# Basant1861/MPC-MMD

Hardware: AMD Instinct MI355X
Metric: MPC optimizer steps/s (batch=1024,H=30,obs_samp=500) @1/2/4/8 GPU; % HBM roofline (higher is better)
Workload: dtype f32; 1 GPU; static obs, mmd_opt, batch=1024 rollouts, H=30, num_obs=10, obs_samples=484 (n=22, M=n^2); cost=mmd_opt, global_batch=1024, num_batch=1024, num_prime=30, num_obs=10, num_reduced=22, noise=gaussian, parallelism=config-sharded x1

## Files before the change

### mpc-mmd_amd/csrc/betacem_common.hpp

```cpp
#pragma once
#include <type_traits>

#include "block.hpp"
#include "kernels.hpp"

namespace mpcmmd {

namespace {

#ifdef MPCMMD_OPAQUE_TIDX
DEVI unsigned tidx() {
  unsigned t = threadIdx.x;
  asm volatile("" : "+v"(t));
  return t;
}
#else
DEVI unsigned tidx() { return threadIdx.x; }
#endif

constexpr int kF = 22;
constexpr int kNew = kBetaSamples - kBetaElite;
constexpr int kThreads = 512;
constexpr double kSqrt20 = 4.47213595499957927704;
constexpr double kRidge = 0.05;
constexpr double kInvRidge = 20.0;

HDI int first_sample(int tb) { return tb > 0 ? kBetaElite : 0; }

#define kconst __attribute__((address_space(4)))
typedef float f2 __attribute__((ext_vector_type(2)));

typedef double d4 __attribute__((ext_vector_type(4)));
DEVI d4 mfma64(double a, double b, d4 c) { return __builtin_amdgcn_mfma_f64_16x16x4f64(a, b, c, 0, 0, 0); }

constexpr int kXcds = 8;
constexpr int kCUs = 256;
constexpr int kKerWaves = 16;
constexpr int kDirWaves = 4;
constexpr int kLptBins = 128;
constexpr double kSeriesAMax = 1.0;
constexpr float kNegLog2e = -1.44269504088896340736f;
constexpr size_t kLdsBudget = 160 * 1024 - 1024;

template <int V = 1, class F>
void with_dist_blocks(int M, F&& f) {
  if constexpr (V == 16) {
    f(std::integral_constant<int, 16>{});
  } else {
    if ((dist_stride(M) >> 8) == V) f(std::integral_constant<int, V>{});
    else with_dist_blocks<V + 1>(M, f);
  }
}

struct LdsTake {
  size_t o = 0;
  HDI size_t operator()(size_t bytes) {
    const size_t at = o;
    o = (o + bytes + 15) & ~size_t(15);
    return at;
  }
};

struct KerLds {
  size_t sel, csg, csd, tri, urank, urow, misc, scratch, total;
};
HDI KerLds ker_lds(int M, int n, size_t scratch) {
  KerLds L{};
  LdsTake take;
  L.sel = take(size_t(kBetaSamples) * n * 2);
  L.csg = take(size_t(kBetaSamples) * 4);
  L.csd = take(size_t(kBetaSamples) * 8);
  L.tri = take(size_t(n) * (n - 1));
  L.urank = take(size_t(M) * 2);
  L.urow = take(size_t(M) * 2);
  L.misc = take(32 * 4);
  L.scratch = take(scratch);
  L.total = take.o;
  return L;
}
HDI size_t ker_sample_bytes(int n) { return size_t(kKerWaves) * n * kFeatStride * 4; }
HDI size_t ker_tab_bytes(int U) { return ((size_t(U) * (U - 1) / 2 * 4 + 15) & ~size_t(15)) + size_t(U) * kFeatStride * 4; }
constexpr size_t kKerTabBytes = 55 * 1024;
constexpr size_t kKerRecBytes = 64 * 1024;
HDI size_t ker_scratch(int M, int n, int tb) {
  size_t sc = ker_sample_bytes(n);
  size_t rec = size_t(M) * kMomStride * 4;
  if (rec > kKerRecBytes) rec = kKerRecBytes;
  if (rec > sc) sc = rec;
  if (tb > 0 && kKerTabBytes > sc) sc = kKerTabBytes;
  return sc;
}

struct DirLds {
  size_t sel, csg, pairs, ulist, ustart, order, bins, misc, scratch, total;
};
HDI DirLds dir_lds(int M, int n) {
  DirLds L{};
  LdsTake take;
  L.sel = take(size_t(kBetaSamples) * n * 2);
  L.csg = take(size_t(kBetaSamples) * 4);
  L.pairs = take(size_t(kBetaSamples) * n * 2);
  L.ulist = take(size_t(M) * 2);
  L.ustart = take(size_t(M + 1) * 2);
  L.order = take(size_t(M) * 2);
  L.bins = take(kLptBins * 4);
  L.misc = take(32 * 4);
  L.scratch = take(size_t(M) * 10);
  L.total = take.o;
  return L;
}

struct EliteLds {
  size_t Gb, misc, carry, ublk, total;
};
constexpr int kUPitch = 12;
HDI EliteLds elite_lds(int M1, int waves = kThreads / 64) {
  EliteLds L{};
  const int nblk = (M1 + 15) / 16;
  L.Gb = 0;
  L.misc = (size_t(nblk) * 66 * 8 + 15) & ~size_t(15);
  L.carry = L.misc + 1024;
  L.ublk = (L.carry + size_t(kBetaElite) * (2 * kMaxReduced + 2) * 4 + 15) & ~size_t(15);
  L.total = L.ublk + size_t(waves) * 16 * kUPitch * 8;
  return L;
}

HDI size_t gen_lds_bytes(int M) { return size_t(pos_pad(M)) * (2 * kGenRow + 1) * 8 + 16 * 8; }
HDI size_t tblk_lds_bytes(int M) { return size_t(pos_pad(M) >> 4) * 4 * 64 * 8; }

}

}
```

### mpc-mmd_amd/csrc/betacem_elite.hpp

```cpp
#pragma once
#include "betacem_common.hpp"

namespace mpcmmd {

namespace {

HDI int sym11(int a, int c) { return a * 11 - a * (a - 1) / 2 + (c - a); }
HDI int sym11i(int a, int c) { return a <= c ? sym11(a, c) : sym11(c, a); }

DEVI void belite_body(const Params& p, int tb, int b, char* smem) {
  const int M = p.M, M1 = M + 1, n = p.n, tid = tidx();
  const EliteLds C = elite_lds(M1, blockDim.x >> 6);
  double* Gb = reinterpret_cast<double*>(smem + C.Gb);
  int* elite = reinterpret_cast<int*>(smem + C.misc);
  int* info = elite + 16;
  float* cst = reinterpret_cast<float*>(info + 16);
  float* sig_new = cst + kBetaSamples;
  uint32_t* ckey = reinterpret_cast<uint32_t*>(sig_new + 12);
  const float* costs = p.bcost + size_t(b) * kBetaSamples;
  if (tid < kBetaSamples) {
    const float c = costs[tid];
    cst[tid] = c;
    ckey[tid] = sort_key(c);
  }
  if (tid == 0) {
    info[0] = -1;
    info[1] = 0;
  }
  __syncthreads();
  if (tid < kBetaSamples) {
    const uint32_t ks = ckey[tid];
    const uint4* k4 = reinterpret_cast<const uint4*>(ckey);
    int r = 0;
#pragma unroll
    for (int k = 0; k < kBetaSamples / 4; ++k) {
      const uint4 v = k4[k];
      r += int(v.x < ks || (v.x == ks && 4 * k < tid)) + int(v.y < ks || (v.y == ks && 4 * k + 1 < tid)) +
           int(v.z < ks || (v.z == ks && 4 * k + 2 < tid)) + int(v.w < ks || (v.w == ks && 4 * k + 3 < tid));
    }
    if (r < kBetaElite) elite[r] = tid;
    if (cst[tid] != cst[tid]) {
      atomicOr(&info[1], 1);
      atomicMin(reinterpret_cast<unsigned*>(&info[0]), unsigned(tid));
    }
  }
  __syncthreads();
  const int imin = info[1] ? info[0] : elite[0];
  if (tid == 0) {
    p.res_beta[size_t(b) * kBetaIters + tb] = info[1] ? __int_as_float(0x7fc00000) : cst[elite[0]];
    double es = 0.0;
    for (int q = 0; q < kBetaElite; ++q) es += double(cst[elite[q]]);
    p.btrace[size_t(b) * kBetaIters + tb] = float(es);
  }
  if (tb < kBetaIters - 1) {
    int* csel = reinterpret_cast<int*>(smem + C.carry);
    float* ctop = reinterpret_cast<float*>(csel + kBetaElite * n);
    float* csig = ctop + kBetaElite * n;
    float* ccost = csig + kBetaElite;
    const size_t rb = size_t(b) * kBetaSamples;
    for (int i = tid; i < kBetaElite * n; i += blockDim.x) {
      const int q = i / n, k = i - q * n;
      const size_t src = (rb + elite[q]) * n + k;
      csel[i] = p.bsel[src];
      ctop[i] = p.btop[src];
    }
    if (tid < kBetaElite) {
      csig[tid] = p.bsig[rb + elite[tid]];
      ccost[tid] = cst[elite[tid]];
    }
    __syncthreads();
    for (int i = tid; i < kBetaElite * n; i += blockDim.x) {
      p.bsel[rb * n + i] = csel[i];
      p.btop[rb * n + i] = ctop[i];
    }
    if (tid < kBetaElite) {
      p.bsig[rb + tid] = csig[tid];
      p.bcost[rb + tid] = ccost[tid];
    }
  }
  const float* Eold = p.belite + (size_t(tb & 1) * p.Bt + b) * kBetaElite * M1;
  float* Enew = p.belite + (size_t((tb + 1) & 1) * p.Bt + b) * kBetaElite * M1;
  const int ys = ygen_stride(M);
  const float* Y = p.ygen + size_t(b) * kBzCols * ys;
  const double rs10 = 1.0 / sqrt(10.0);
  double* gen = p.gen + size_t(b) * pos_pad(M) * kGenStride;
  const int nblk = (M1 + 15) / 16;
  const int span = ((nblk * 16 + 63) / 64) * 64;
  for (int j = tid; j < span; j += blockDim.x) {
    const bool valid = j < M1;
    double u[kBetaElite], mean;
    {
      float v[kBetaElite];
      double s = 0.0;
      const int jc = min(j, M);
#pragma unroll
      for (int q = 0; q < kBetaElite; ++q) {
        const int e = elite[q];
        const float* src = tb == 0 ? p.beta_z0 + size_t(e) * M1
                                   : (e < kBetaElite ? Eold + size_t(e) * M1 : Y + size_t(e - kBetaElite) * ys);
        v[q] = src[jc];
      }
#pragma unroll
      for (int q = 0; q < kBetaElite; ++q) {
        float x = v[q];
        if (tb == 0) {
          x = float(kSqrt20 * double(x));
          if (j == M) x = fmaxf(x, 0.01f);
        }
        x = valid ? x : 0.0f;
        if (valid) {
          Enew[size_t(q) * M1 + j] = x;
          if (j == M) sig_new[q] = x;
        }
        v[q] = x;
        s = s + double(x);
      }
      const double m = s / double(kBetaElite);
#pragma unroll
      for (int q = 0; q < kBetaElite; ++q) u[q] = valid ? (double(v[q]) - m) * rs10 : 0.0;
      mean = valid ? double(float(m)) : 0.0;
    }
    double* ub = reinterpret_cast<double*>(smem + C.ublk) + (tid >> 6) * 16 * kUPitch;
    const int lane = tid & 63, r = lane & 15, h = lane >> 4;
#pragma unroll
    for (int k = 0; k < 4; ++k) {
      const int blk = (j >> 6) * 4 + k;
      if ((lane >> 4) == k) {
#pragma unroll
        for (int q = 0; q < kBetaElite; ++q) ub[(lane & 15) * kUPitch + q] = u[q];
        ub[(lane & 15) * kUPitch + kGenMean] = mean;
      }
      wave_sync();
      d4 G = d4{0.0, 0.0, 0.0, 0.0};
#pragma unroll
      for (int st = 0; st < 4; ++st) {
        const double x = r < 11 ? ub[(4 * st + h) * kUPitch + r] : 0.0;
        G = mfma64(x, x, G);
      }
#pragma unroll
      for (int i = 0; i < 3; ++i) {
        const int e = lane + 64 * i, row = e / kGenRow, q = e - row * kGenRow;
        const int pos = blk * 16 + row;
        if (pos < M1) gen[gen_uplane(pos_pad(M)) + size_t(pos) * kGenRow + q] = ub[row * kUPitch + q];
      }
      wave_sync();
#pragma unroll
      for (int i = 0; i < 4; ++i) {
        const int a = h + 4 * i;
        if (blk < nblk && a <= r && r < 11) Gb[blk * 66 + sym11(a, r)] = G[i];
      }
    }
  }
  __syncthreads();
  if (tid < 66) {
    int a = 0, c = tid;
    while (c >= 11 - a) {
      c -= 11 - a;
      ++a;
    }
    c += a;
    double acc = a == c ? 1.0 : 0.0;
    double* ph = p.phib + size_t(b) * nblk * 66;
#pragma unroll 8
    for (int blk = 0; blk < nblk; ++blk) {
      const double g = Gb[blk * 66 + tid];
      ph[blk * 66 + tid] = acc;
      acc = fma(g, kInvRidge, acc);
    }
  }
  if (tb == kBetaIters - 1) {
    const int* bsel = p.bsel + (size_t(b) * kBetaSamples + imin) * n;
    for (int i = tid; i < n; i += blockDim.x) {
      p.bestsel[size_t(b) * n + i] = bsel[i];
      p.beta[size_t(b) * n + i] = p.btop[(size_t(b) * kBetaSamples + imin) * n + i];
    }
    if (tid == 0) {
      p.bimin[b] = imin;
      if (imin < kBetaElite) p.sigma[b] = sig_new[imin];
    }
  }
}

DEVI double rcp_nr(double d) {
  double y = __builtin_amdgcn_rcp(d);
  y = fma(y, fma(-d, y, 1.0), y);
  return fma(y, fma(-d, y, 1.0), y);
}
DEVI double rsq_nr(double d) {
  double y = __builtin_amdgcn_rsq(d);
#pragma unroll
  for (int it = 0; it < 2; ++it) {
    const double e = fma(-(d * y), y, 1.0);
    y = fma(0.5 * y, e, y);
  }
  return y;
}

DEVI void bgen_wave(const Params& p, int b, int blk, double* xl) {
  const int M = p.M, M1 = M + 1, nblk = (M1 + 15) / 16, Pp = pos_pad(M);
  const int lane = tidx() & 63, r = lane & 15, h = lane >> 4;
  double* gen = p.gen + size_t(b) * Pp * kGenStride;
  double* gm = p.genm + size_t(b) * Pp;
  const int j0 = blk * 16;
  d4 A;
  double U[3];
  const double* Gb = p.phib + (size_t(b) * nblk + blk) * 66;
#pragma unroll
  for (int i = 0; i < 4; ++i) {
    const int a = h + 4 * i;
    A[i] = a < 11 && r < 11 ? Gb[sym11i(min(a, 10), min(r, 10))] : 0.0;
  }
#pragma unroll
  for (int s = 0; s < 3; ++s) {
    const int f = 4 * s + h;
    U[s] = f < 11 && j0 + r < M1 ? gen[gen_uplane(Pp) + size_t(j0 + r) * kGenRow + f] : 0.0;
  }
#pragma unroll
  for (int k = 0; k < 11; ++k) {
    if (r == k) {
#pragma unroll
      for (int i = 0; i < 4; ++i) xl[h + 4 * i] = A[i];
    }
    wave_sync();
    const double d = xl[k], cr = xl[r];
    double ci[4];
#pragma unroll
    for (int i = 0; i < 4; ++i) ci[i] = xl[h + 4 * i];
    wave_sync();
    const double id = rcp_nr(d);
#pragma unroll
    for (int i = 0; i < 4; ++i) {
      const int a = h + 4 * i;
      A[i] = a == k ? (r == k ? -id : cr * id) : (r == k ? ci[i] * id : A[i] - (ci[i] * cr) * id);
    }
  }
  const d4 zero = d4{0.0, 0.0, 0.0, 0.0};
#pragma unroll
  for (int i = 0; i < 4; ++i) A[i] = -A[i];
  d4 V = zero, G = zero;
#pragma unroll
  for (int s = 0; s < 3; ++s) V = mfma64(A[s], U[s], V);
#pragma unroll
  for (int s = 0; s < 3; ++s) G = mfma64(U[s], V[s], G);
#pragma unroll
  for (int i = 0; i < 4; ++i)
    if (h + 4 * i == r) G[i] = G[i] + kRidge;
#pragma unroll
  for (int k = 0; k < 16; ++k) {
    if (r == k) {
#pragma unroll
      for (int i = 0; i < 4; ++i) {
        xl[h + 4 * i] = G[i];
        xl[16 + h + 4 * i] = V[i];
      }
    }
    wave_sync();
    const double d = xl[k], gr = xl[r];
    double gi[4], vi[4];
#pragma unroll
    for (int i = 0; i < 4; ++i) {
      gi[i] = xl[h + 4 * i];
      vi[i] = xl[16 + h + 4 * i];
    }
    wave_sync();
    const double rl = rsq_nr(d);
    const double lr = r > k ? gr * rl : 0.0;
    double wk[4];
#pragma unroll
    for (int i = 0; i < 4; ++i) {
      const double li = h + 4 * i > k ? gi[i] * rl : 0.0;
      wk[i] = vi[i] * rl;
      G[i] = G[i] - li * lr;
      V[i] = V[i] - wk[i] * lr;
    }
    const int j = j0 + k;
    if (r == k && j < M1) {
      double* g = gen + size_t(j) * kGenRow + kGenW;
#pragma unroll
      for (int i = 0; i < 3; ++i) g[h + 4 * i] = h + 4 * i < 11 ? wk[i] : 0.0;
      if (h == 0) gm[j] = d * rl;
    }
  }
}

DEVI void bsigma_body(const Params& p, int tb, int b, double* red) {
  const int M = p.M, tid = tidx();
  const int imin = p.bimin[b];
  const double* gen = p.gen + size_t(b) * pos_pad(M) * kGenStride;
  {
    const float* z = p.beta_z + size_t(tb) * pos_pad(M) * kBzCols;
    const int si = imin - kBetaElite;
    double part[11];
#pragma unroll
    for (int a = 0; a < 11; ++a) part[a] = 0.0;
    for (int j = tid; j < M && tid < kThreads; j += kThreads) {
      const double zj = double(z[bz_index(j, si)]);
#pragma unroll
      for (int a = 0; a < 11; ++a) part[a] += gen[size_t(j) * kGenRow + kGenW + a] * zj;
    }
#pragma unroll
    for (int a = 0; a < 11; ++a) {
      part[a] = wave_total(part[a]);
    }
    __syncthreads();
    if ((tid & 63) == 0 && tid < kThreads)
#pragma unroll
      for (int a = 0; a < 11; ++a) red[(tid >> 6) * 11 + a] = part[a];
    __syncthreads();
    if (tid == 0) {
      const double* g = gen + size_t(M) * kGenRow;
      const double* gu = g + gen_uplane(pos_pad(M));
      double d = 0.0;
      for (int a = 0; a < 11; ++a) {
        double sa = 0.0;
        for (int w2 = 0; w2 < kThreads / 64; ++w2) sa += red[w2 * 11 + a];
        d += gu[a] * sa;
      }
      const double zM = z[bz_index(M, si)];
      const float yM = float((gu[kGenMean] + p.genm[size_t(b) * pos_pad(M) + M] * zM) + d);
      p.sigma[b] = fmaxf(yM, 0.01f);
    }
  }
}

}

}
```

### mpc-mmd_amd/csrc/betacem_sample.hpp

```cpp
#pragma once
#include "betacem_common.hpp"

namespace mpcmmd {

namespace {

constexpr int kSampleTiles = kBzCols / 16;
static_assert(kBzCols >= kNew, "sample tiles");
constexpr int kChunkWavesMax = 12;
HDI int sample_chunk(int nblk) {
  int cl = nblk <= 8 ? 4 : 8;
  while ((nblk + cl - 1) / cl > kChunkWavesMax) cl <<= 1;
  return cl;
}
template <int TPW>
constexpr int sample_waves() {
  static_assert(kSampleTiles % TPW == 0, "tiles per wave");
  return kSampleTiles / TPW;
}

template <int TPW>
struct SampleBlock {
  double wA[4];
  double wX[3];
  double uX[3];
  double L;
  float z[TPW][4];
};

template <int TPW>
DEVI void load_block(SampleBlock<TPW>& q, const double* G, const double* GU, const double* gm, const float* z, int p0,
                     int s0, int r, int h) {
#pragma unroll
  for (int k = 0; k < 4; ++k) q.wA[k] = G[size_t(p0 + 4 * k + h) * kGenRow + kGenW + r];
  const double* g = G + size_t(p0 + r) * kGenRow;
  const double* gu = GU + size_t(p0 + r) * kGenRow;
#pragma unroll
  for (int i = 0; i < 3; ++i) {
    q.wX[i] = g[kGenW + 4 * i + h];
    q.uX[i] = gu[4 * i + h];
  }
  q.L = gm[p0 + r];
  static_assert(TPW == 1 || TPW == kSampleTiles, "tile pairing of the normals' layout");
  if constexpr (TPW == 1) {
#pragma unroll
    for (int k = 0; k < 4; ++k) q.z[0][k] = z[bz_index(p0 + 4 * k + h, s0 + r)];
  } else {
    const float4* zb = reinterpret_cast<const float4*>(z + size_t(p0 >> 4) * (16 * kBzCols)) + r + 16 * h;
#pragma unroll
    for (int c = 0; c < 6; ++c) {
      const float4 f = zb[64 * c];
      const float fv[4] = {f.x, f.y, f.z, f.w};
#pragma unroll
      for (int w = 0; w < 4; ++w) {
        const int idx = 4 * c + w, k = idx / 6, t = idx % 6;
        q.z[t][k] = fv[w];
      }
    }
  }
}

struct SampleRsrc {
  __amdgpu_buffer_rsrc_t gen, genm, z;
  int vA, vX, vL, vZ;
  int uplane;
};
DEVI SampleRsrc sample_rsrc(const double* G, const double* gm, const float* z, int Pp, int r, int h) {
  SampleRsrc s;
  s.gen = __builtin_amdgcn_make_buffer_rsrc(const_cast<double*>(G), short(0), Pp * kGenStride * 8, 0x00020000);
  s.genm = __builtin_amdgcn_make_buffer_rsrc(const_cast<double*>(gm), short(0), Pp * 8, 0x00020000);
  s.z = __builtin_amdgcn_make_buffer_rsrc(const_cast<float*>(z), short(0), Pp * kBzCols * 4, 0x00020000);
  s.vA = (h * kGenRow + kGenW + r) * 8;
  s.vX = (r * kGenRow + h) * 8;
  s.vL = r * 8;
  s.vZ = (r + 16 * h) * 16;
  s.uplane = Pp * kGenRow * 8;
  return s;
}
DEVI double buf_ld_d(__amdgpu_buffer_rsrc_t rs, int voff, int soff) {
  return __builtin_bit_cast(double, __builtin_amdgcn_raw_buffer_load_b64(rs, voff, soff, 0));
}
DEVI void load_block_buf(SampleBlock<kSampleTiles>& q, const SampleRsrc& s, int p0) {
  const int sg = p0 * kGenRow * 8;
#pragma unroll
  for (int k = 0; k < 4; ++k) q.wA[k] = buf_ld_d(s.gen, s.vA + k * 4 * kGenRow * 8, sg);
#pragma unroll
  for (int i = 0; i < 3; ++i) {
    q.wX[i] = buf_ld_d(s.gen, s.vX + 32 * i, sg);
    q.uX[i] = buf_ld_d(s.gen, s.vX + 32 * i, sg + s.uplane);
  }
  q.L = buf_ld_d(s.genm, s.vL, p0 * 8);
  const int szz = (p0 >> 4) * (16 * kBzCols * 4);
#pragma unroll
  for (int c = 0; c < 6; ++c) {
    typedef float v4f __attribute__((ext_vector_type(4)));
    const v4f f = __builtin_bit_cast(v4f, __builtin_amdgcn_raw_buffer_load_b128(s.z, s.vZ + 1024 * (c % 3), szz + 3072 * (c / 3), 0));
#pragma unroll
    for (int w = 0; w < 4; ++w) {
      const int idx = 4 * c + w, k = idx / 6, t = idx % 6;
      q.z[t][k] = f[w];
    }
  }
}

template <int TPW>
DEVI void block_mfma(const SampleBlock<TPW>& cur, d4* S, const d4* Sp, d4* Y, int r, int h) {
  double zd[TPW][4];
#pragma unroll
  for (int t = 0; t < TPW; ++t)
#pragma unroll
    for (int k = 0; k < 4; ++k) zd[t][k] = double(cur.z[t][k]);
  d4 X = d4{0.0, 0.0, 0.0, 0.0};
#pragma unroll
  for (int i = 0; i < 3; ++i) X = mfma64(cur.wX[i], cur.uX[i], X);
  const d4 zero = d4{0.0, 0.0, 0.0, 0.0};
  double St[TPW][3];
#pragma unroll
  for (int t = 0; t < TPW; ++t)
#pragma unroll
    for (int k = 0; k < 3; ++k) St[t][k] = Sp[t][k] + S[t][k];
#pragma unroll
  for (int k = 0; k < 3; ++k)
#pragma unroll
    for (int t = 0; t < TPW; ++t) Y[t] = mfma64(St[t][k], cur.uX[k], k == 0 ? zero : Y[t]);
#pragma unroll
  for (int k = 0; k < 4; ++k)
#pragma unroll
    for (int t = 0; t < TPW; ++t) S[t] = mfma64(cur.wA[k], zd[t][k], S[t]);
  double T[4];
#pragma unroll
  for (int i = 0; i < 4; ++i) {
    const int k = h + 4 * i;
    T[i] = k < r ? X[i] : (k == r ? cur.L : 0.0);
  }
#pragma unroll
  for (int k = 0; k < 4; ++k)
#pragma unroll
    for (int t = 0; t < TPW; ++t) Y[t] = mfma64(zd[t][k], T[k], Y[t]);
}

HDI_CONST int tile_sample(int TPW, int s0, int t, int rho) { return TPW == 1 ? s0 + rho : 32 * (t >> 1) + 2 * rho + (t & 1); }
template <int TPW>
DEVI void block_store(const d4* Yv, float* plane, int p0, int M, int ys, int s0, int r, int h) {
  if (p0 > M) return;
#pragma unroll
  for (int t = 0; t < TPW; ++t)
#pragma unroll
    for (int i = 0; i < 4; ++i) {
      const int s = tile_sample(TPW, s0, t, h + 4 * i);
      const float v = float(Yv[t][i]);
      if (s < kNew) plane[size_t(s) * ys + p0 + r] = p0 + r == M ? fmaxf(v, 0.01f) : v;
    }
}

DEVI __amdgpu_buffer_rsrc_t ygen_rsrc(float* plane, int ys) {
  return __builtin_amdgcn_make_buffer_rsrc(plane, short(0), kBzCols * ys * 4, 0x00020000);
}
constexpr int kDropOffset = 0x7FFFFF00;
static_assert(kNew == 89, "tile 4 / 5 register 3 validity below");
DEVI void block_store_rows(const d4* Yv, __amdgpu_buffer_rsrc_t yr, int p0, int ys, int vl, int v43) {
#pragma unroll
  for (int t = 0; t < kSampleTiles; ++t)
#pragma unroll
    for (int i = 0; i < 4; ++i) {
      if (t == 5 && i == 3) continue;
      const int soff = ((32 * (t >> 1) + (t & 1) + 8 * i) * ys + p0) * 4;
      __builtin_amdgcn_raw_buffer_store_b32(__float_as_uint(float(Yv[t][i])), yr, t == 4 && i == 3 ? v43 : vl, soff, 0);
    }
}

DEVI void fold_chunk(d4& Sp, d4& S) {
#pragma unroll
  for (int k = 0; k < 3; ++k) Sp[k] = Sp[k] + S[k];
  S = d4{0.0, 0.0, 0.0, 0.0};
}

constexpr int kZAhead = 4;

DEVI void bsample_tblocks(const Params& p, const double* lg, double* Tl, int w, int W) {
  const int M = p.M, Pp = pos_pad(M), nblk = Pp >> 4;
  const int lane = tidx() & 63, r = lane & 15, h = lane >> 4;
  for (int blk = w; blk < nblk; blk += W) {
    const int p0 = blk * 16;
    const double* g = lg + size_t(p0 + r) * kGenRow;
    const double* gu = lg + gen_uplane(Pp) + size_t(p0 + r) * kGenRow;
    double wX[3], uX[3];
#pragma unroll
    for (int i = 0; i < 3; ++i) {
      wX[i] = g[kGenW + 4 * i + h];
      uX[i] = gu[4 * i + h];
    }
    const double L = lg[2 * gen_uplane(Pp) + p0 + r];
    d4 X = d4{0.0, 0.0, 0.0, 0.0};
#pragma unroll
    for (int i = 0; i < 3; ++i) X = mfma64(wX[i], uX[i], X);
#pragma unroll
    for (int i = 0; i < 4; ++i) {
      const int k = h + 4 * i;
      Tl[(size_t(blk) * 4 + i) * 64 + lane] = k < r ? X[i] : (k == r ? L : 0.0);
    }
  }
}

DEVI void bsample_unit_lds(const Params& p, int tb, int b, int tile, int chunk, const double* lg, const double* Tl) {
  const int M = p.M, Pp = pos_pad(M), nblk = Pp >> 4, cl = sample_chunk(nblk);
  const int c0 = chunk * cl, c1 = min(nblk, c0 + cl);
  const int lane = tidx() & 63, r = lane & 15, h = lane >> 4, s0 = tile * 16;
  const double* LW = lg;
  const double* LU = lg + gen_uplane(Pp);
  const float* z = p.beta_z + size_t(tb - 1) * Pp * kBzCols;
  const int ys = ygen_stride(M);
  float* plane = p.ygen + size_t(b) * kBzCols * ys;
  d4 S = d4{0.0, 0.0, 0.0, 0.0}, Sp = d4{0.0, 0.0, 0.0, 0.0};
  Sp[2] = h == 3 ? 1.0 : 0.0;
  auto zload = [&](float (&zz)[4], int c) {
#pragma unroll
    for (int k = 0; k < 4; ++k) zz[k] = z[bz_index(c * 16 + 4 * k + h, s0 + r)];
  };
  float zr[kZAhead][4];
#pragma unroll
  for (int u = 0; u < kZAhead; ++u) zload(zr[u], min(u, c1 - 1));
  const d4 zero = d4{0.0, 0.0, 0.0, 0.0};
  for (int c = 0; c < c1; c += kZAhead) {
#pragma unroll
    for (int u = 0; u < kZAhead; ++u) {
      const int cb = c + u;
      if (cb < c1) {
        const int p0 = cb * 16;
        double zd[4], wA[4];
#pragma unroll
        for (int k = 0; k < 4; ++k) {
          zd[k] = double(zr[u][k]);
          wA[k] = LW[size_t(p0 + 4 * k + h) * kGenRow + kGenW + r];
        }
        zload(zr[u], min(cb + kZAhead, c1 - 1));
        if (cb >= c0) {
          double uX[3], T[4];
#pragma unroll
          for (int i = 0; i < 3; ++i) uX[i] = LU[size_t(p0 + r) * kGenRow + 4 * i + h];
#pragma unroll
          for (int i = 0; i < 4; ++i) T[i] = Tl[(size_t(cb) * 4 + i) * 64 + lane];
          double St[3];
#pragma unroll
          for (int k = 0; k < 3; ++k) St[k] = Sp[k] + S[k];
          d4 Y = zero;
#pragma unroll
          for (int k = 0; k < 3; ++k) Y = mfma64(St[k], uX[k], k == 0 ? zero : Y);
#pragma unroll
          for (int k = 0; k < 4; ++k) S = mfma64(wA[k], zd[k], S);
#pragma unroll
          for (int k = 0; k < 4; ++k) Y = mfma64(zd[k], T[k], Y);
          block_store<1>(&Y, plane, p0, M, ys, s0, r, h);
        } else {
#pragma unroll
          for (int k = 0; k < 4; ++k) S = mfma64(wA[k], zd[k], S);
        }
        if ((cb + 1) % cl == 0) fold_chunk(Sp, S);
      }
    }
  }
}

}

}
```

### mpc-mmd_amd/csrc/k_bcem_small.hip

```cpp
#define MPCMMD_OPAQUE_TIDX 1
#include "betacem_elite.hpp"
#include "betacem_kernel.hpp"
#include "betacem_qp.hpp"
#include "betacem_sample.hpp"
#include "betacem_select.hpp"

namespace mpcmmd {

namespace {

constexpr int kSmallWaves = kKerWaves, kSmallThreads = 64 * kSmallWaves;
constexpr int kSmallSelR = 1, kSmallSelG = 32;
constexpr size_t kSmallCandBytes = size_t(64 * kSmallSelR + 8) * 8;
constexpr size_t kSmallSelBytes = kSmallCandBytes + 64 * 4 + 128 * 4;
HDI size_t small_lds(int M, int n) {
  size_t b = kSmallWaves * kSmallSelBytes + size_t(kNew) * ygen_stride(M) * 4;
  const size_t k = ker_lds(M, n, ker_scratch(M, n, 1)).total;
  const size_t d = dir_lds(M, n).total, e = elite_lds(M + 1, kSmallWaves).total;
  const size_t q = (size_t(kBetaSamples) * tri_stride(n) + kQpZeros) * 4;
  const size_t gl = ((gen_lds_bytes(M) + 15) & ~size_t(15)) + tblk_lds_bytes(M);
  b = b > q ? b : q;
  b = b > gl ? b : gl;
  b = b > k ? b : k;
  b = b > d ? b : d;
  b = b > e ? b : e;
  return b;
}

HDI size_t small_persist_off(int M, int n) { return (small_lds(M, n) + 15) & ~size_t(15); }
HDI size_t small_persist_bytes(int M) { return size_t(M) * (kMomStride + kFeatStride) * 4; }

#define SMALL_STAMP(p, slot)                                                             \
  do {                                                                                   \
    if (tidx() == 0 && (p).dbgw)                                                    \
      (p).dbgw[size_t(32768 + blockIdx.x) * 8 + (slot)] = __builtin_amdgcn_s_memrealtime(); \
  } while (0)

template <int NQ, int NP>
__global__ __launch_bounds__(kSmallThreads) void k_bcem_small(Params p0, int persist) {
  extern __shared__ __attribute__((aligned(16))) char smem[];
  const int cand = blockIdx.x;
  const int tid = tidx();
  const int w = __builtin_amdgcn_readfirstlane(tid >> 6);
  const float4* mom_l = nullptr;
  const float4* feat_l = nullptr;
  if (persist) {
    const int M = p0.M, b = p0.b0 + cand;
    float4* pm = reinterpret_cast<float4*>(smem + small_persist_off(M, p0.n));
    float4* pf = pm + M * (kMomStride / 4);
    const float4* gm = reinterpret_cast<const float4*>(p0.bmom + size_t(b) * M * kMomStride);
    const float4* gf = reinterpret_cast<const float4*>(p0.featr + size_t(b) * M * kFeatStride);
    for (int i = tid; i < M * (kMomStride / 4); i += kSmallThreads) pm[i] = gm[i];
    for (int i = tid; i < M * (kFeatStride / 4); i += kSmallThreads) pf[i] = gf[i];
    mom_l = pm;
    feat_l = pf;
    __syncthreads();
  }
  for (int tb = 0; tb < kBetaIters; ++tb) {
    typedef const Params __attribute__((address_space(4)))* KParams;
    KParams pk = (KParams)__builtin_amdgcn_kernarg_segment_ptr();
    asm volatile("" : "+s"(pk));
    const Params& p = *(const Params*)pk;
    const int b = p.b0 + cand, M = p.M, n = p.n;
    const int ntri = tri_stride(n);
    if (tb > 0) {
      if (tb == 5) SMALL_STAMP(p, 0);
      {
        const int Pp = pos_pad(M);
        const double2* gsrc = reinterpret_cast<const double2*>(p.gen + size_t(b) * Pp * kGenStride);
        const double2* msrc = reinterpret_cast<const double2*>(p.genm + size_t(b) * Pp);
        double2* dst = reinterpret_cast<double2*>(smem);
        const int ng = Pp * kGenRow, nm = Pp >> 1;
        for (int i = tid; i < ng + nm; i += kSmallThreads) dst[i] = i < ng ? gsrc[i] : msrc[i - ng];
        if (tid < 8) dst[ng + nm + tid] = double2{0.0, 0.0};
      }
      __syncthreads();
      {
        const double* lg = reinterpret_cast<const double*>(smem);
        double* Tl = reinterpret_cast<double*>(smem + ((gen_lds_bytes(M) + 15) & ~size_t(15)));
        bsample_tblocks(p, lg, Tl, w, kSmallWaves);
        __syncthreads();
        const int nblk = pos_pad(M) >> 4, units = kSampleTiles * ((nblk + sample_chunk(nblk) - 1) / sample_chunk(nblk));
        for (int u = w; u < units; u += kSmallWaves) bsample_unit_lds(p, tb, b, u % kSampleTiles, u / kSampleTiles, lg, Tl);
      }
      __syncthreads();
      if (tb == 5) SMALL_STAMP(p, 1);
      const int ys = ygen_stride(M);
      const float* Yl = reinterpret_cast<const float*>(smem + kSmallWaves * kSmallSelBytes);
      {
        const float4* src = reinterpret_cast<const float4*>(p.ygen + size_t(b) * kBzCols * ys);
        float4* dst = reinterpret_cast<float4*>(smem + kSmallWaves * kSmallSelBytes);
        for (int i = tid; i < kNew * (ys >> 2); i += kSmallThreads) dst[i] = src[i];
      }
      __syncthreads();
      char* sw = smem + size_t(w) * kSmallSelBytes;
      unsigned long long* cand_l = reinterpret_cast<unsigned long long*>(sw);
      uint32_t* lm = reinterpret_cast<uint32_t*>(sw + kSmallCandBytes);
      int* scr = reinterpret_cast<int*>(sw + kSmallCandBytes + 64 * 4);
      {
        int32_t* sel = p.bsel + size_t(b) * kBetaSamples * n;
        float* sig = p.bsig + size_t(b) * kBetaSamples;
        auto row = [&](int s) {
          const float* r = Yl + size_t(s - kBetaElite) * ys;
          return [=](int j) { return r[j]; };
        };
        const int s_lo = first_sample(tb), lane = tid & 63;
        if (s_lo + w < kBetaSamples) {
          select_walk<NQ, kSmallSelR, kSmallSelG>(row, [&](int s) { return sel + s * n; }, s_lo + w, kBetaSamples,
                                                  kSmallWaves, M, n, cand_l, lm, scr);
          for (int s2 = s_lo + w + lane * kSmallWaves; lane < 16 && s2 < kBetaSamples; s2 += 16 * kSmallWaves)
            sig[s2] = row(s2)(M);
        }
      }
    } else {
      for (int e = tid; e < kBetaSamples * n; e += kSmallThreads) p.bsel[size_t(b) * kBetaSamples * n + e] = p.sel0[e];
      for (int e = tid; e < kBetaSamples; e += kSmallThreads) p.bsig[size_t(b) * kBetaSamples + e] = p.sig0[e];
    }
    __syncthreads();
    if (tb == 5) SMALL_STAMP(p, 2);
    bkernel_body<false, true>(p, tb, cand, 0, 1, int(ker_scratch(M, n, tb)), smem, mom_l, feat_l);
    __syncthreads();
    if (tb == 5) SMALL_STAMP(p, 3);
    if (tb > 0) {
      const int total = bdirect_total(p, b, 1);
      if (total > 0) {
        bdirect_body<1, kSmallWaves>(p, tb, 1, 1, cand, 0, total, smem);
        __syncthreads();
      }
    }
    if (tb == 5) SMALL_STAMP(p, 4);
    {
      const int s_lo = first_sample(tb), per = kBetaSamples - s_lo;
      const float4* src = reinterpret_cast<const float4*>(p.bkred + (size_t(b) * kBetaSamples + s_lo) * ntri);
      float4* kl4 = reinterpret_cast<float4*>(smem);
      for (int i = tid; i < per * (ntri >> 2); i += kSmallThreads) kl4[i] = src[i];
      if (tid < kQpZeros) reinterpret_cast<float*>(smem)[per * ntri + tid] = 0.0f;
      __syncthreads();
      static_assert(kSmallThreads / 4 >= kBetaSamples, "one quad per QP");
      const int g = tid >> 2;
      const bool ok = g < per;
      const int gc = ok ? g : 0;
      bqp_solve<NP>(p, b, s_lo + gc, ok, reinterpret_cast<const float*>(smem) + size_t(gc) * ntri,
                    reinterpret_cast<const float*>(smem) + size_t(per) * ntri);
    }
    __syncthreads();
    if (tb == 5) SMALL_STAMP(p, 5);
    belite_body(p, tb, b, smem);
    __syncthreads();
    if (tb == 5) SMALL_STAMP(p, 6);
    {
      const int nblk = (M + 1 + 15) / 16;
      double* xl = reinterpret_cast<double*>(smem) + 32 * w;
      for (int blk = w; blk < nblk; blk += kSmallWaves) bgen_wave(p, b, blk, xl);
    }
    __syncthreads();
    if (tb == 5) SMALL_STAMP(p, 7);
    if (tb == kBetaIters - 1 && p.bimin[b] >= kBetaElite) {
      bsigma_body(p, tb, b, reinterpret_cast<double*>(smem));
      __syncthreads();
    }
  }
}

}

bool bcem_small_ok(const Params& p) {
  return p.gen_wave && p.M <= 256 && p.nb <= 512 && small_lds(p.M, p.n) <= kLdsBudget;
}

void launch_bcem_small(const Params& p, hipStream_t s) {
  const int n = p.n, M = p.M;
  const dim3 grid(p.nb), block(kSmallThreads);
  const size_t lp = small_persist_off(M, n) + small_persist_bytes(M);
  const int persist = lp <= kLdsBudget;
  const size_t lds = persist ? lp : small_lds(M, n);
  if (M <= 64)
    hipLaunchKernelGGL((k_bcem_small<1, 8>), grid, block, lds, s, p, persist);
  else if (M <= 128)
    hipLaunchKernelGGL((k_bcem_small<2, 12>), grid, block, lds, s, p, persist);
  else
    hipLaunchKernelGGL((k_bcem_small<4, 16>), grid, block, lds, s, p, persist);
}

}
```

### mpc-mmd_amd/csrc/k_belite.hip

```cpp
#include "betacem_elite.hpp"

namespace mpcmmd {

namespace {

__global__ __launch_bounds__(kThreads) void k_belite(Params p, int tb) {
  extern __shared__ __attribute__((aligned(16))) char smem[];
  belite_body(p, tb, p.b0 + blockIdx.x, smem);
}

DEVI void bgen_quad(const Params& p, int b, int blk, bool live) {
  const int M = p.M, M1 = M + 1, nblk = (M1 + 15) / 16;
  const int q = tidx() & 3;
  double* gen = p.gen + size_t(b) * pos_pad(M) * kGenStride;
  const double* Gb = p.phib + (size_t(b) * nblk + blk) * 66;
  double A[3][11];
#pragma unroll
  for (int i = 0; i < 3; ++i) {
    const int a = q + 4 * i;
#pragma unroll
    for (int c = 0; c < 11; ++c) A[i][c] = a < 11 ? Gb[sym11i(a, c)] : 0.0;
  }
#pragma unroll
  for (int k = 0; k < 11; ++k) {
    const int ik = k >> 2, ok = k & 3;
    const double ip = 1.0 / quad_bcast(A[ik][k], ok);
    double f[3];
#pragma unroll
    for (int i = 0; i < 3; ++i) f[i] = A[i][k];
#pragma unroll
    for (int c = 0; c < 11; ++c) {
      const double rc = c == k ? ip : quad_bcast(A[ik][c], ok) * ip;
#pragma unroll
      for (int i = 0; i < 3; ++i) {
        const bool pivot_row = q + 4 * i == k;
        A[i][c] = pivot_row ? rc : (c == k ? -f[i] * ip : fma(-f[i], rc, A[i][c]));
      }
    }
  }
  const int j0 = blk * 16, j1 = min(M1, j0 + 16);
  double un[11];
  double uon[3];
  const double* ub = gen + gen_uplane(pos_pad(M));
#pragma unroll
  for (int c = 0; c < 11; ++c) un[c] = ub[size_t(j0) * kGenRow + c];
#pragma unroll
  for (int i = 0; i < 3; ++i) uon[i] = ub[size_t(j0) * kGenRow + q + 4 * i];
  for (int j = j0; j < j1; ++j) {
    double u[11], uo[3];
#pragma unroll
    for (int c = 0; c < 11; ++c) u[c] = un[c];
#pragma unroll
    for (int i = 0; i < 3; ++i) uo[i] = uon[i];
    const int jn = min(j + 1, j1 - 1);
#pragma unroll
    for (int c = 0; c < 11; ++c) un[c] = ub[size_t(jn) * kGenRow + c];
#pragma unroll
    for (int i = 0; i < 3; ++i) uon[i] = ub[size_t(jn) * kGenRow + q + 4 * i];
    double v[3], part = 0.0;
#pragma unroll
    for (int i = 0; i < 3; ++i) {
      double s = 0.0;
#pragma unroll
      for (int c = 0; c < 11; ++c) s = fma(A[i][c], u[c], s);
      v[i] = s;
      const int a = q + 4 * i;
      part = fma(i < 2 || a < 11 ? uo[i] : 0.0, s, part);
    }
    const double uv = quad_sum(part);
    const double ljj = sqrt(kRidge + uv);
    const double rl = 1.0 / ljj;
    double w[3];
#pragma unroll
    for (int i = 0; i < 3; ++i) w[i] = v[i] * rl;
    double* g = gen + size_t(j) * kGenRow;
    if (live) {
#pragma unroll
      for (int i = 0; i < 3; ++i) g[kGenW + q + 4 * i] = q + 4 * i < 11 ? w[i] : 0.0;
      if (q == 0) p.genm[size_t(b) * pos_pad(M) + j] = ljj;
    }
#pragma unroll
    for (int c = 0; c < 11; ++c) {
      const double wc = quad_bcast(w[c >> 2], c & 3);
#pragma unroll
      for (int i = 0; i < 3; ++i) A[i][c] = fma(-w[i], wc, A[i][c]);
    }
  }
}

__global__ __launch_bounds__(256) __attribute__((amdgpu_waves_per_eu(2))) void k_bgen(Params p) {
  const int nblk = (p.M + 1 + 15) / 16;
  const int gq = (blockIdx.x * blockDim.x + tidx()) >> 2;
  const bool live = gq < p.nb * nblk;
  const int gqc = live ? gq : p.nb * nblk - 1;
  bgen_quad(p, p.b0 + gqc / nblk, gqc % nblk, live);
}

constexpr int kGenWaveWaves = 4;
__global__ __launch_bounds__(64 * kGenWaveWaves) void k_bgen_wave(Params p) {
  __shared__ double xl[kGenWaveWaves][32];
  const int nblk = (p.M + 1 + 15) / 16;
  const int w = tidx() >> 6, gw = blockIdx.x * kGenWaveWaves + w;
  if (gw >= p.nb * nblk) return;
  bgen_wave(p, p.b0 + gw / nblk, gw % nblk, xl[w]);
}

__global__ __launch_bounds__(kThreads) void k_bsigma(Params p, int tb) {
  __shared__ double red[(kThreads / 64) * 11];
  const int b = p.b0 + blockIdx.x;
  if (p.bimin[b] < kBetaElite) return;
  bsigma_body(p, tb, b, red);
}

}

void launch_belite(const Params& p, int tb, hipStream_t s) {
  const EliteLds e = elite_lds(p.M + 1);
  hipLaunchKernelGGL(k_belite, dim3(p.nb), dim3(kThreads), e.total, s, p, tb);
}

void launch_bgen(const Params& p, int tb, hipStream_t s) {
  const int nblk = (p.M + 1 + 15) / 16;
  if (p.gen_wave)
    hipLaunchKernelGGL(k_bgen_wave, dim3((p.nb * nblk + kGenWaveWaves - 1) / kGenWaveWaves), dim3(64 * kGenWaveWaves), 0,
                       s, p);
  else
    hipLaunchKernelGGL(k_bgen, dim3((p.nb * nblk * 4 + 255) / 256), dim3(256), 0, s, p);
  if (tb == kBetaIters - 1) hipLaunchKernelGGL(k_bsigma, dim3(p.nb), dim3(kThreads), 0, s, p, tb);
}

}
```

### mpc-mmd_amd/csrc/k_bsample.hip

```cpp
#include <algorithm>

#include "betacem_sample.hpp"
#include "betacem_select.hpp"

namespace mpcmmd {

namespace {

__global__ __launch_bounds__(256) void k_bsel0(Params p) {
  const int n = p.n, per = kBetaSamples * n + kBetaSamples;
  for (size_t x = size_t(blockIdx.x) * 256 + tidx(); x < size_t(p.nb) * per; x += size_t(gridDim.x) * 256) {
    const int c = int(x / per), e = int(x - size_t(c) * per), b = p.b0 + c;
    if (e < kBetaSamples * n)
      p.bsel[size_t(b) * kBetaSamples * n + e] = p.sel0[e];
    else
      p.bsig[size_t(b) * kBetaSamples + e - kBetaSamples * n] = p.sig0[e - kBetaSamples * n];
  }
}

template <int TPW>
__global__ __launch_bounds__(64 * sample_waves<TPW>()) void k_bsample(Params p, int tb) {
  const int b = p.b0 + blockIdx.x, M = p.M, Pp = pos_pad(M);
  const int lane = tidx() & 63, w = tidx() >> 6;
  const int r = lane & 15, h = lane >> 4;
  const int s0 = w * TPW * 16;
  MPCMMD_STAMP(p, 0);
  const double* G = p.gen + size_t(b) * Pp * kGenStride;
  const double* gm = p.genm + size_t(b) * Pp;
  const float* z = p.beta_z + size_t(tb - 1) * Pp * kBzCols;
  const int ys = ygen_stride(M);
  float* plane = p.ygen + size_t(b) * kBzCols * ys;
  d4 S[TPW], Sp[TPW], Ya[TPW], Yb[TPW];
#pragma unroll
  for (int t = 0; t < TPW; ++t) {
    S[t] = Sp[t] = d4{0.0, 0.0, 0.0, 0.0};
    Sp[t][2] = h == 3 ? 1.0 : 0.0;
  }
  const int nblk = Pp >> 4, cl = sample_chunk(nblk);
  const __amdgpu_buffer_rsrc_t yr = ygen_rsrc(plane, ys);
  const int vl = (2 * h * ys + r) * 4, v43 = h == 0 ? vl : kDropOffset;
  auto store = [&](const d4* Yv, int q0) {
    if (TPW == kSampleTiles && q0 + 15 < M)
      block_store_rows(Yv, yr, q0, ys, vl, v43);
    else
      block_store<TPW>(Yv, plane, q0, M, ys, s0, r, h);
  };
  SampleBlock<TPW> qa, qb;
  const SampleRsrc srs = sample_rsrc(G, gm, z, Pp, r, h);
  auto load = [&](SampleBlock<TPW>& q, int q0) {
    if constexpr (TPW == kSampleTiles)
      load_block_buf(q, srs, q0);
    else
      load_block(q, G, G + gen_uplane(Pp), gm, z, q0, s0, r, h);
  };
  load(qa, 0);
  for (int c = 0; c < nblk; c += 2) {
    const int p0 = c << 4;
    load(qb, p0 + 16);
    __builtin_amdgcn_sched_barrier(0);
    block_mfma(qa, S, Sp, Ya, r, h);
    __builtin_amdgcn_sched_barrier(0);
    if (c > 0) store(Yb, p0 - 16);
    __builtin_amdgcn_sched_barrier(0);
    load(qa, min(p0 + 32, Pp - 16));
    __builtin_amdgcn_sched_barrier(0);
    block_mfma(qb, S, Sp, Yb, r, h);
    if ((c + 2) % cl == 0)
#pragma unroll
      for (int t = 0; t < TPW; ++t) fold_chunk(Sp[t], S[t]);
    __builtin_amdgcn_sched_barrier(0);
    store(Ya, p0);
    __builtin_amdgcn_sched_barrier(0);
  }
  store(Yb, Pp - 16);
  MPCMMD_STAMP(p, 1);
}

__global__ __launch_bounds__(64 * kChunkWavesMax) void k_bsample_chunks(Params p, int tb) {
  __shared__ double dS[kChunkWavesMax - 1][3][64];
  const int b = p.b0 + blockIdx.x, M = p.M, Pp = pos_pad(M), nblk = Pp >> 4;
  const int lane = tidx() & 63, k = tidx() >> 6, P = blockDim.x >> 6;
  const int r = lane & 15, h = lane >> 4, s0 = blockIdx.y * 16;
  const int cl = sample_chunk(nblk), c0 = k * cl, c1 = min(nblk, c0 + cl);
  MPCMMD_STAMP(p, 0);
  const double* G = p.gen + size_t(b) * Pp * kGenStride;
  const double* gm = p.genm + size_t(b) * Pp;
  const float* z = p.beta_z + size_t(tb - 1) * Pp * kBzCols;
  const int ys = ygen_stride(M);
  float* plane = p.ygen + size_t(b) * kBzCols * ys;
  if (k < P - 1) {
    auto ld = [&](double (&wa)[4], double (&zz)[4], int c) {
#pragma unroll
      for (int kk = 0; kk < 4; ++kk) {
        const size_t pos = size_t(c) * 16 + 4 * kk + h;
        wa[kk] = G[pos * kGenRow + kGenW + r];
        zz[kk] = double(z[bz_index(int(pos), s0 + r)]);
      }
    };
    d4 Sl = d4{0.0, 0.0, 0.0, 0.0};
    double wa[4], zz[4], wn[4], zn[4];
    ld(wa, zz, c0);
    for (int c = c0; c < c1; ++c) {
      ld(wn, zn, min(c + 1, c1 - 1));
#pragma unroll
      for (int kk = 0; kk < 4; ++kk) Sl = mfma64(wa[kk], zz[kk], Sl);
#pragma unroll
      for (int kk = 0; kk < 4; ++kk) {
        wa[kk] = wn[kk];
        zz[kk] = zn[kk];
      }
    }
#pragma unroll
    for (int i = 0; i < 3; ++i) dS[k][i][lane] = Sl[i];
  }
  __syncthreads();
  d4 S[1] = {d4{0.0, 0.0, 0.0, 0.0}}, Sp[1] = {d4{0.0, 0.0, 0.0, 0.0}}, Ya[1], Yb[1];
  Sp[0][2] = h == 3 ? 1.0 : 0.0;
  for (int j = 0; j < k; ++j)
#pragma unroll
    for (int i = 0; i < 3; ++i) Sp[0][i] = Sp[0][i] + dS[j][i][lane];
  SampleBlock<1> qa, qb;
  const int pend = c1 << 4;
  load_block(qa, G, G + gen_uplane(Pp), gm, z, c0 << 4, s0, r, h);
  for (int c = c0; c < c1; c += 2) {
    const int p0 = c << 4;
    load_block(qb, G, G + gen_uplane(Pp), gm, z, p0 + 16, s0, r, h);
    __builtin_amdgcn_sched_barrier(0);
    block_mfma(qa, S, Sp, Ya, r, h);
    __builtin_amdgcn_sched_barrier(0);
    if (c > c0) block_store<1>(Yb, plane, p0 - 16, M, ys, s0, r, h);
    __builtin_amdgcn_sched_barrier(0);
    load_block(qa, G, G + gen_uplane(Pp), gm, z, min(p0 + 32, pend - 16), s0, r, h);
    __builtin_amdgcn_sched_barrier(0);
    block_mfma(qb, S, Sp, Yb, r, h);
    __builtin_amdgcn_sched_barrier(0);
    block_store<1>(Ya, plane, p0, M, ys, s0, r, h);
    __builtin_amdgcn_sched_barrier(0);
  }
  block_store<1>(Yb, plane, pend - 16, M, ys, s0, r, h);
  MPCMMD_STAMP(p, 1);
}

template <int NQ, int R, int G>
__global__ __launch_bounds__(64) void k_bselect(Params p, int tb) {
  __shared__ __attribute__((aligned(16))) unsigned long long cand[64 * R + 8];
  __shared__ __attribute__((aligned(16))) uint32_t lm[64];
  __shared__ int scratch[128];
  if (blockIdx.y == 0 && tidx() == 0) p.bdlcount[size_t(p.b0 + blockIdx.x) * kBetaIters + tb] = 0;
  bselect_wave<NQ, R, G>(p, tb, p.b0 + blockIdx.x, blockIdx.y, gridDim.y, cand, lm, scratch);
}

}

void launch_bsample(const Params& p, int tb, hipStream_t s) {
  if (p.nb >= 384) {
    hipLaunchKernelGGL((k_bsample<6>), dim3(p.nb), dim3(64 * sample_waves<6>()), 0, s, p, tb);
  } else {
    const int nblk = pos_pad(p.M) >> 4, cl = sample_chunk(nblk);
    hipLaunchKernelGGL(k_bsample_chunks, dim3(p.nb, kSampleTiles), dim3(64 * ((nblk + cl - 1) / cl)), 0, s, p, tb);
  }
}

void launch_bsel0(const Params& p, hipStream_t s) {
  const size_t total = size_t(p.nb) * (kBetaSamples * p.n + kBetaSamples);
  hipLaunchKernelGGL(k_bsel0, dim3(unsigned(std::min<size_t>((total + 255) / 256, 4096))), dim3(256), 0, s, p);
}

int sel_waves(int nb, int cap) { return std::max(4, std::min(nb <= 128 ? cap : 16, 16384 / std::max(1, nb))); }

template <int NQ, int R, int G>
void launch_bselect_i(const Params& p, int tb, hipStream_t s) {
  hipLaunchKernelGGL((k_bselect<NQ, R, G>), dim3(p.nb, sel_waves(p.nb, p.sel_cap)), dim3(64), 0, s, p, tb);
}

void launch_bselect(const Params& p, int tb, hipStream_t s) {
  const int n = p.n;
  if (n <= 8) return launch_bselect_i<1, 1, 32>(p, tb, s);
  if (n <= 11) return launch_bselect_i<2, 1, 32>(p, tb, s);
  if (n <= 16) return launch_bselect_i<4, 1, 32>(p, tb, s);
  if (n <= 22) return launch_bselect_i<8, 1, 32>(p, tb, s);
  if (n <= 24) return launch_bselect_i<12, 1, 32>(p, tb, s);
  if (n <= 27) return launch_bselect_i<12, 2, 64>(p, tb, s);
  if (n <= 32) return launch_bselect_i<16, 2, 64>(p, tb, s);
  if (n <= 39) return launch_bselect_i<24, 2, 64>(p, tb, s);
  if (n <= 45) return launch_bselect_i<32, 2, 64>(p, tb, s);
  if (n <= 48) return launch_bselect_i<40, 2, 64>(p, tb, s);
  if (n <= 50) return launch_bselect_i<40, 2, 0>(p, tb, s);
  if (n <= 55) return launch_bselect_i<48, 2, 0>(p, tb, s);
  return launch_bselect_i<64, 2, 0>(p, tb, s);
}

}
```

### mpc-mmd_amd/csrc/layout.hpp

```cpp
#pragma once
#include <cstddef>

#ifdef __HIPCC__
#define HDI_CONST __host__ __device__ __forceinline__ constexpr
#else
#define HDI_CONST inline constexpr
#endif

namespace mpcmmd {

constexpr int kMaxH = 100;
constexpr int kMaxReduced = 64;
constexpr int kBetaSamples = 100;
constexpr int kBetaIters = 20;
constexpr int kBetaElite = 11;
constexpr int kEliteCost = 20;
constexpr int kCnormStride = 12;
constexpr int kElite = 5;
constexpr int kResultStride = 11 + 11 + 2 + 1 + 20 + kMaxReduced;
constexpr int kGenRow = 12;
constexpr int kGenStride = 2 * kGenRow;
constexpr int kGenW = 0, kGenMean = 11;
HDI_CONST size_t gen_uplane(int Pp) { return size_t(Pp) * kGenRow; }
HDI_CONST int ygen_stride(int M) { return ((M + 1) + 31) & ~31; }
constexpr int kBzCols = 96;
HDI_CONST size_t bz_index(int j, int s) {
  const int jj = j & 15, lane = ((s & 31) >> 1) + 16 * (jj & 3), idx = 6 * (jj >> 2) + 2 * (s >> 5) + (s & 1);
  return size_t(j >> 4) * (16 * kBzCols) + (idx >> 2) * 256 + lane * 4 + (idx & 3);
}
HDI_CONST int pos_pad(int M) { return ((M + 1) + 31) & ~31; }
HDI_CONST int dist_stride(int M) { return (M + 255) & ~255; }
HDI_CONST int tri_stride(int n) { return ((n * (n - 1) / 2) + 3) & ~3; }
constexpr int kFeatStride = 24;
constexpr int kMom = 12;
constexpr int kMomStride = 16;
constexpr int kMomR = 12;
HDI_CONST size_t gtab_stride(int S, int H) { return size_t(4) * 4 * 4 * S * H; }
constexpr int kMaxSplit = 8;
constexpr int kMaxPath = 2048;
constexpr int kMaxDetObs = 32;

}
```

Measured before the change: 140.7 steps/s.

## Recompute centered elite U on the fly instead of storing double U plane

The elite kernel no longer writes the 12-wide double U plane to global memory. It writes only a per-position mean row. Consumers (gen, sample, sigma, small kernel) reload the float elites plus the mean and recompute u = (e - m)/sqrt(10) in registers, which cuts global write and read traffic roughly in half. The sample loops are also refactored into a shared walk_blocks helper that handles the tail block explicitly, and bgen_quad stages elites through LDS with 128-bit buffer loads. The cost is extra FLOPs and more scattered strided float loads across the elite rows.

```diff
diff --git a/mpc-mmd_amd/csrc/betacem_common.hpp b/mpc-mmd_amd/csrc/betacem_common.hpp
--- a/mpc-mmd_amd/csrc/betacem_common.hpp
+++ b/mpc-mmd_amd/csrc/betacem_common.hpp
@@ -26,6 +26,20 @@
 constexpr double kInvRidge = 20.0;
 
 HDI int first_sample(int tb) { return tb > 0 ? kBetaElite : 0; }
+
+DEVI const float* gen_elites(const Params& p, int half, int b) {
+  return p.belite + (size_t(half & 1) * p.Bt + b) * kBetaElite * (p.M + 1);
+}
+DEVI const double* gen_mean_row(const Params& p, int b) {
+  return p.gen + size_t(b) * pos_pad(p.M) * kGenStride + gen_means(pos_pad(p.M));
+}
+
+DEVI float buf_ld_f(__amdgpu_buffer_rsrc_t rs, int voff, int soff) {
+  return __builtin_bit_cast(float, __builtin_amdgcn_raw_buffer_load_b32(rs, voff, soff, 0));
+}
+DEVI double buf_ld_d(__amdgpu_buffer_rsrc_t rs, int voff, int soff) {
+  return __builtin_bit_cast(double, __builtin_amdgcn_raw_buffer_load_b64(rs, voff, soff, 0));
+}
 
 #define kconst __attribute__((address_space(4)))
 typedef float f2 __attribute__((ext_vector_type(2)));
@@ -125,6 +139,7 @@
   return L;
 }
 
+HDI size_t lds_uplane(int Pp) { return size_t(Pp) * kGenRow; }
 HDI size_t gen_lds_bytes(int M) { return size_t(pos_pad(M)) * (2 * kGenRow + 1) * 8 + 16 * 8; }
 HDI size_t tblk_lds_bytes(int M) { return size_t(pos_pad(M) >> 4) * 4 * 64 * 8; }
 
diff --git a/mpc-mmd_amd/csrc/betacem_elite.hpp b/mpc-mmd_amd/csrc/betacem_elite.hpp
--- a/mpc-mmd_amd/csrc/betacem_elite.hpp
+++ b/mpc-mmd_amd/csrc/betacem_elite.hpp
@@ -82,13 +82,12 @@
   float* Enew = p.belite + (size_t((tb + 1) & 1) * p.Bt + b) * kBetaElite * M1;
   const int ys = ygen_stride(M);
   const float* Y = p.ygen + size_t(b) * kBzCols * ys;
-  const double rs10 = 1.0 / sqrt(10.0);
-  double* gen = p.gen + size_t(b) * pos_pad(M) * kGenStride;
+  double* gmean = p.gen + size_t(b) * pos_pad(M) * kGenStride + gen_means(pos_pad(M));
   const int nblk = (M1 + 15) / 16;
   const int span = ((nblk * 16 + 63) / 64) * 64;
   for (int j = tid; j < span; j += blockDim.x) {
     const bool valid = j < M1;
-    double u[kBetaElite], mean;
+    double u[kBetaElite];
     {
       float v[kBetaElite];
       double s = 0.0;
@@ -117,8 +116,8 @@
       }
       const double m = s / double(kBetaElite);
 #pragma unroll
-      for (int q = 0; q < kBetaElite; ++q) u[q] = valid ? (double(v[q]) - m) * rs10 : 0.0;
-      mean = valid ? double(float(m)) : 0.0;
+      for (int q = 0; q < kBetaElite; ++q) u[q] = valid ? gen_u(v[q], m) : 0.0;
+      if (valid) gmean[j] = m;
     }
     double* ub = reinterpret_cast<double*>(smem + C.ublk) + (tid >> 6) * 16 * kUPitch;
     const int lane = tid & 63, r = lane & 15, h = lane >> 4;
@@ -128,7 +127,6 @@
       if ((lane >> 4) == k) {
 #pragma unroll
         for (int q = 0; q < kBetaElite; ++q) ub[(lane & 15) * kUPitch + q] = u[q];
-        ub[(lane & 15) * kUPitch + kGenMean] = mean;
       }
       wave_sync();
       d4 G = d4{0.0, 0.0, 0.0, 0.0};
@@ -136,12 +134,6 @@
       for (int st = 0; st < 4; ++st) {
         const double x = r < 11 ? ub[(4 * st + h) * kUPitch + r] : 0.0;
         G = mfma64(x, x, G);
-      }
-#pragma unroll
-      for (int i = 0; i < 3; ++i) {
-        const int e = lane + 64 * i, row = e / kGenRow, q = e - row * kGenRow;
-        const int pos = blk * 16 + row;
-        if (pos < M1) gen[gen_uplane(pos_pad(M)) + size_t(pos) * kGenRow + q] = ub[row * kUPitch + q];
       }
       wave_sync();
 #pragma unroll
@@ -196,7 +188,7 @@
   return y;
 }
 
-DEVI void bgen_wave(const Params& p, int b, int blk, double* xl) {
+DEVI void bgen_wave(const Params& p, int tb, int b, int blk, double* xl) {
   const int M = p.M, M1 = M + 1, nblk = (M1 + 15) / 16, Pp = pos_pad(M);
   const int lane = tidx() & 63, r = lane & 15, h = lane >> 4;
   double* gen = p.gen + size_t(b) * Pp * kGenStride;
@@ -205,15 +197,19 @@
   d4 A;
   double U[3];
   const double* Gb = p.phib + (size_t(b) * nblk + blk) * 66;
+  const float* E = gen_elites(p, tb + 1, b);
 #pragma unroll
   for (int i = 0; i < 4; ++i) {
     const int a = h + 4 * i;
     A[i] = a < 11 && r < 11 ? Gb[sym11i(min(a, 10), min(r, 10))] : 0.0;
   }
+  const int jr = min(j0 + r, M);
+  const double mr = gen_mean_row(p, b)[jr];
 #pragma unroll
   for (int s = 0; s < 3; ++s) {
     const int f = 4 * s + h;
-    U[s] = f < 11 && j0 + r < M1 ? gen[gen_uplane(Pp) + size_t(j0 + r) * kGenRow + f] : 0.0;
+    const float e = E[size_t(min(f, 10)) * M1 + jr];
+    U[s] = f < 11 && j0 + r < M1 ? gen_u(e, mr) : 0.0;
   }
 #pragma unroll
   for (int k = 0; k < 11; ++k) {
@@ -308,16 +304,16 @@
       for (int a = 0; a < 11; ++a) red[(tid >> 6) * 11 + a] = part[a];
     __syncthreads();
     if (tid == 0) {
-      const double* g = gen + size_t(M) * kGenRow;
-      const double* gu = g + gen_uplane(pos_pad(M));
+      const float* EM = gen_elites(p, tb + 1, b) + M;
+      const double mM = gen_mean_row(p, b)[M];
       double d = 0.0;
       for (int a = 0; a < 11; ++a) {
         double sa = 0.0;
         for (int w2 = 0; w2 < kThreads / 64; ++w2) sa += red[w2 * 11 + a];
-        d += gu[a] * sa;
+        d += gen_u(EM[size_t(a) * (M + 1)], mM) * sa;
       }
       const double zM = z[bz_index(M, si)];
-      const float yM = float((gu[kGenMean] + p.genm[size_t(b) * pos_pad(M) + M] * zM) + d);
+      const float yM = float((gen_mean_slot(mM) + p.genm[size_t(b) * pos_pad(M) + M] * zM) + d);
       p.sigma[b] = fmaxf(yM, 0.01f);
     }
   }
diff --git a/mpc-mmd_amd/csrc/betacem_sample.hpp b/mpc-mmd_amd/csrc/betacem_sample.hpp
--- a/mpc-mmd_amd/csrc/betacem_sample.hpp
+++ b/mpc-mmd_amd/csrc/betacem_sample.hpp
@@ -13,6 +13,7 @@
   while ((nblk + cl - 1) / cl > kChunkWavesMax) cl <<= 1;
   return cl;
 }
+HDI int sample_blocks(int M) { return (M + 1 + 15) >> 4; }
 template <int TPW>
 constexpr int sample_waves() {
   static_assert(kSampleTiles % TPW == 0, "tiles per wave");
@@ -23,23 +24,32 @@
 struct SampleBlock {
   double wA[4];
   double wX[3];
-  double uX[3];
+  float eX[3];
+  double m;
   double L;
   float z[TPW][4];
 };
 
+template <bool TAIL, int TPW>
+DEVI void block_u(const SampleBlock<TPW>& q, double (&uX)[3], int h, bool valid) {
+#pragma unroll
+  for (int i = 0; i < 3; ++i) uX[i] = gen_u(TAIL && !valid ? 0.0f : q.eX[i], q.m);
+  uX[2] = h == 3 ? gen_mean_slot(q.m) : uX[2];
+}
+
 template <int TPW>
-DEVI void load_block(SampleBlock<TPW>& q, const double* G, const double* GU, const double* gm, const float* z, int p0,
-                     int s0, int r, int h) {
+DEVI void load_block(SampleBlock<TPW>& q, const double* G, const float* E, const double* mrow, const double* gm,
+                     const float* z, int M, int p0, int s0, int r, int h) {
 #pragma unroll
   for (int k = 0; k < 4; ++k) q.wA[k] = G[size_t(p0 + 4 * k + h) * kGenRow + kGenW + r];
   const double* g = G + size_t(p0 + r) * kGenRow;
-  const double* gu = GU + size_t(p0 + r) * kGenRow;
+  const float* e = E + min(p0 + r, M);
 #pragma unroll
   for (int i = 0; i < 3; ++i) {
     q.wX[i] = g[kGenW + 4 * i + h];
-    q.uX[i] = gu[4 * i + h];
-  }
+    q.eX[i] = e[size_t(min(4 * i + h, kBetaElite - 1)) * (M + 1)];
+  }
+  q.m = mrow[p0 + r];
   q.L = gm[p0 + r];
   static_assert(TPW == 1 || TPW == kSampleTiles, "tile pairing of the normals' layout");
   if constexpr (TPW == 1) {
@@ -61,24 +71,26 @@
 }
 
 struct SampleRsrc {
-  __amdgpu_buffer_rsrc_t gen, genm, z;
-  int vA, vX, vL, vZ;
-  int uplane;
+  __amdgpu_buffer_rsrc_t gen, genm, z, el;
+  int vA, vX, vL, vZ, vE;
+  int means;
+  int erow;
 };
-DEVI SampleRsrc sample_rsrc(const double* G, const double* gm, const float* z, int Pp, int r, int h) {
+DEVI SampleRsrc sample_rsrc(const double* G, const float* E, const double* gm, const float* z, int M, int r, int h) {
   SampleRsrc s;
+  const int Pp = pos_pad(M);
   s.gen = __builtin_amdgcn_make_buffer_rsrc(const_cast<double*>(G), short(0), Pp * kGenStride * 8, 0x00020000);
+  s.el = __builtin_amdgcn_make_buffer_rsrc(const_cast<float*>(E), short(0), kBetaElite * (M + 1) * 4, 0x00020000);
   s.genm = __builtin_amdgcn_make_buffer_rsrc(const_cast<double*>(gm), short(0), Pp * 8, 0x00020000);
   s.z = __builtin_amdgcn_make_buffer_rsrc(const_cast<float*>(z), short(0), Pp * kBzCols * 4, 0x00020000);
   s.vA = (h * kGenRow + kGenW + r) * 8;
   s.vX = (r * kGenRow + h) * 8;
   s.vL = r * 8;
   s.vZ = (r + 16 * h) * 16;
-  s.uplane = Pp * kGenRow * 8;
+  s.vE = (h * (M + 1) + r) * 4;
+  s.means = int(gen_means(Pp)) * 8;
+  s.erow = 4 * (M + 1) * 4;
   return s;
-}
-DEVI double buf_ld_d(__amdgpu_buffer_rsrc_t rs, int voff, int soff) {
-  return __builtin_bit_cast(double, __builtin_amdgcn_raw_buffer_load_b64(rs, voff, soff, 0));
 }
 DEVI void load_block_buf(SampleBlock<kSampleTiles>& q, const SampleRsrc& s, int p0) {
   const int sg = p0 * kGenRow * 8;
@@ -87,8 +99,9 @@
 #pragma unroll
   for (int i = 0; i < 3; ++i) {
     q.wX[i] = buf_ld_d(s.gen, s.vX + 32 * i, sg);
-    q.uX[i] = buf_ld_d(s.gen, s.vX + 32 * i, sg + s.uplane);
-  }
+    q.eX[i] = buf_ld_f(s.el, s.vE, p0 * 4 + i * s.erow);
+  }
+  q.m = buf_ld_d(s.gen, s.vL, p0 * 8 + s.means);
   q.L = buf_ld_d(s.genm, s.vL, p0 * 8);
   const int szz = (p0 >> 4) * (16 * kBzCols * 4);
 #pragma unroll
@@ -103,8 +116,10 @@
   }
 }
 
-template <int TPW>
-DEVI void block_mfma(const SampleBlock<TPW>& cur, d4* S, const d4* Sp, d4* Y, int r, int h) {
+template <bool TAIL = false, int TPW>
+DEVI void block_mfma(const SampleBlock<TPW>& cur, d4* S, const d4* Sp, d4* Y, int r, int h, bool valid = true) {
+  double uX[3];
+  block_u<TAIL>(cur, uX, h, valid);
   double zd[TPW][4];
 #pragma unroll
   for (int t = 0; t < TPW; ++t)
@@ -112,7 +127,7 @@
     for (int k = 0; k < 4; ++k) zd[t][k] = double(cur.z[t][k]);
   d4 X = d4{0.0, 0.0, 0.0, 0.0};
 #pragma unroll
-  for (int i = 0; i < 3; ++i) X = mfma64(cur.wX[i], cur.uX[i], X);
+  for (int i = 0; i < 3; ++i) X = mfma64(cur.wX[i], uX[i], X);
   const d4 zero = d4{0.0, 0.0, 0.0, 0.0};
   double St[TPW][3];
 #pragma unroll
@@ -122,7 +137,7 @@
 #pragma unroll
   for (int k = 0; k < 3; ++k)
 #pragma unroll
-    for (int t = 0; t < TPW; ++t) Y[t] = mfma64(St[t][k], cur.uX[k], k == 0 ? zero : Y[t]);
+    for (int t = 0; t < TPW; ++t) Y[t] = mfma64(St[t][k], uX[k], k == 0 ? zero : Y[t]);
 #pragma unroll
   for (int k = 0; k < 4; ++k)
 #pragma unroll
@@ -175,22 +190,67 @@
   S = d4{0.0, 0.0, 0.0, 0.0};
 }
 
+template <int TPW, class Load, class Store, class PairEnd>
+DEVI void walk_blocks(int c0, int c1, int M, int r, int h, d4* S, const d4* Sp, Load&& load, Store&& store,
+                      PairEnd&& pair_end) {
+  d4 Ya[TPW], Yb[TPW];
+  SampleBlock<TPW> qa, qb;
+  const int last = c1 - 1;
+  const bool valid = (last << 4) + r <= M;
+  load(qa, c0 << 4);
+  int c = c0;
+  for (; c + 2 <= last; c += 2) {
+    const int p0 = c << 4;
+    load(qb, p0 + 16);
+    __builtin_amdgcn_sched_barrier(0);
+    block_mfma(qa, S, Sp, Ya, r, h);
+    __builtin_amdgcn_sched_barrier(0);
+    if (c > c0) store(Yb, p0 - 16);
+    __builtin_amdgcn_sched_barrier(0);
+    load(qa, p0 + 32);
+    __builtin_amdgcn_sched_barrier(0);
+    block_mfma(qb, S, Sp, Yb, r, h);
+    pair_end(c);
+    __builtin_amdgcn_sched_barrier(0);
+    store(Ya, p0);
+    __builtin_amdgcn_sched_barrier(0);
+  }
+  const int p0 = c << 4;
+  if (c < last) {
+    load(qb, p0 + 16);
+    __builtin_amdgcn_sched_barrier(0);
+    block_mfma(qa, S, Sp, Ya, r, h);
+    __builtin_amdgcn_sched_barrier(0);
+    if (c > c0) store(Yb, p0 - 16);
+    __builtin_amdgcn_sched_barrier(0);
+    block_mfma<true>(qb, S, Sp, Yb, r, h, valid);
+    __builtin_amdgcn_sched_barrier(0);
+    store(Ya, p0);
+    store(Yb, p0 + 16);
+  } else {
+    block_mfma<true>(qa, S, Sp, Ya, r, h, valid);
+    __builtin_amdgcn_sched_barrier(0);
+    if (c > c0) store(Yb, p0 - 16);
+    store(Ya, p0);
+  }
+}
+
 constexpr int kZAhead = 4;
 
 DEVI void bsample_tblocks(const Params& p, const double* lg, double* Tl, int w, int W) {
-  const int M = p.M, Pp = pos_pad(M), nblk = Pp >> 4;
+  const int M = p.M, Pp = pos_pad(M), nblk = sample_blocks(M);
   const int lane = tidx() & 63, r = lane & 15, h = lane >> 4;
   for (int blk = w; blk < nblk; blk += W) {
     const int p0 = blk * 16;
     const double* g = lg + size_t(p0 + r) * kGenRow;
-    const double* gu = lg + gen_uplane(Pp) + size_t(p0 + r) * kGenRow;
+    const double* gu = lg + lds_uplane(Pp) + size_t(p0 + r) * kGenRow;
     double wX[3], uX[3];
 #pragma unroll
     for (int i = 0; i < 3; ++i) {
       wX[i] = g[kGenW + 4 * i + h];
       uX[i] = gu[4 * i + h];
     }
-    const double L = lg[2 * gen_uplane(Pp) + p0 + r];
+    const double L = lg[2 * lds_uplane(Pp) + p0 + r];
     d4 X = d4{0.0, 0.0, 0.0, 0.0};
 #pragma unroll
     for (int i = 0; i < 3; ++i) X = mfma64(wX[i], uX[i], X);
@@ -203,11 +263,11 @@
 }
 
 DEVI void bsample_unit_lds(const Params& p, int tb, int b, int tile, int chunk, const double* lg, const double* Tl) {
-  const int M = p.M, Pp = pos_pad(M), nblk = Pp >> 4, cl = sample_chunk(nblk);
-  const int c0 = chunk * cl, c1 = min(nblk, c0 + cl);
+  const int M = p.M, Pp = pos_pad(M), cl = sample_chunk(Pp >> 4);
+  const int c0 = chunk * cl, c1 = min(sample_blocks(M), c0 + cl);
   const int lane = tidx() & 63, r = lane & 15, h = lane >> 4, s0 = tile * 16;
   const double* LW = lg;
-  const double* LU = lg + gen_uplane(Pp);
+  const double* LU = lg + lds_uplane(Pp);
   const float* z = p.beta_z + size_t(tb - 1) * Pp * kBzCols;
   const int ys = ygen_stride(M);
   float* plane = p.ygen + size_t(b) * kBzCols * ys;
diff --git a/mpc-mmd_amd/csrc/k_bcem_small.hip b/mpc-mmd_amd/csrc/k_bcem_small.hip
--- a/mpc-mmd_amd/csrc/k_bcem_small.hip
+++ b/mpc-mmd_amd/csrc/k_bcem_small.hip
@@ -66,12 +66,21 @@
     if (tb > 0) {
       if (tb == 5) SMALL_STAMP(p, 0);
       {
-        const int Pp = pos_pad(M);
+        const int Pp = pos_pad(M), M1 = M + 1;
         const double2* gsrc = reinterpret_cast<const double2*>(p.gen + size_t(b) * Pp * kGenStride);
         const double2* msrc = reinterpret_cast<const double2*>(p.genm + size_t(b) * Pp);
         double2* dst = reinterpret_cast<double2*>(smem);
-        const int ng = Pp * kGenRow, nm = Pp >> 1;
-        for (int i = tid; i < ng + nm; i += kSmallThreads) dst[i] = i < ng ? gsrc[i] : msrc[i - ng];
+        const int nw = Pp * (kGenRow / 2), ng = 2 * nw, nm = Pp >> 1;
+        for (int i = tid; i < nw + nm; i += kSmallThreads) dst[i < nw ? i : i + nw] = i < nw ? gsrc[i] : msrc[i - nw];
+        const float* E = gen_elites(p, tb, b);
+        const double* mrow = gen_mean_row(p, b);
+        double* ul = reinterpret_cast<double*>(smem) + lds_uplane(Pp);
+        for (int i = tid; i < Pp * kGenRow; i += kSmallThreads) {
+          const int pos = i / kGenRow, q = i - pos * kGenRow;
+          const double m = mrow[pos];
+          const float e = pos < M1 ? E[min(q, kBetaElite - 1) * M1 + pos] : 0.0f;
+          ul[i] = q < kBetaElite ? gen_u(e, m) : gen_mean_slot(m);
+        }
         if (tid < 8) dst[ng + nm + tid] = double2{0.0, 0.0};
       }
       __syncthreads();
@@ -151,7 +160,7 @@
     {
       const int nblk = (M + 1 + 15) / 16;
       double* xl = reinterpret_cast<double*>(smem) + 32 * w;
-      for (int blk = w; blk < nblk; blk += kSmallWaves) bgen_wave(p, b, blk, xl);
+      for (int blk = w; blk < nblk; blk += kSmallWaves) bgen_wave(p, tb, b, blk, xl);
     }
     __syncthreads();
     if (tb == 5) SMALL_STAMP(p, 7);
diff --git a/mpc-mmd_amd/csrc/k_belite.hip b/mpc-mmd_amd/csrc/k_belite.hip
--- a/mpc-mmd_amd/csrc/k_belite.hip
+++ b/mpc-mmd_amd/csrc/k_belite.hip
@@ -9,10 +9,32 @@
   belite_body(p, tb, p.b0 + blockIdx.x, smem);
 }
 
-DEVI void bgen_quad(const Params& p, int b, int blk, bool live) {
+constexpr int kGenStage = 16 * 12 + 4;
+DEVI void bgen_quad(const Params& p, int tb, int b, int blk, bool live, float* st) {
   const int M = p.M, M1 = M + 1, nblk = (M1 + 15) / 16;
   const int q = tidx() & 3;
   double* gen = p.gen + size_t(b) * pos_pad(M) * kGenStride;
+  const int j0 = blk * 16, j1 = min(M1, j0 + 16);
+  {
+    typedef float v4f __attribute__((ext_vector_type(4)));
+    const __amdgpu_buffer_rsrc_t er = __builtin_amdgcn_make_buffer_rsrc(
+        const_cast<float*>(gen_elites(p, tb + 1, p.b0)), short(0), p.nb * kBetaElite * M1 * 4, 0x00020000);
+    const int vb = ((b - p.b0) * kBetaElite * M1 + j0) * 4;
+    v4f f[3][4];
+#pragma unroll
+    for (int i = 0; i < 3; ++i)
+#pragma unroll
+      for (int k = 0; k < 4; ++k)
+        f[i][k] = __builtin_bit_cast(
+            v4f, __builtin_amdgcn_raw_buffer_load_b128(er, vb + (min(q + 4 * i, 10) * M1 + 4 * k) * 4, 0, 0));
+#pragma unroll
+    for (int i = 0; i < 3; ++i)
+#pragma unroll
+      for (int k = 0; k < 4; ++k)
+#pragma unroll
+        for (int w = 0; w < 4; ++w) st[(4 * k + w) * 12 + q + 4 * i] = q + 4 * i < 11 ? f[i][k][w] : 0.0f;
+    wave_sync();
+  }
   const double* Gb = p.phib + (size_t(b) * nblk + blk) * 66;
   double A[3][11];
 #pragma unroll
@@ -38,25 +60,30 @@
       }
     }
   }
-  const int j0 = blk * 16, j1 = min(M1, j0 + 16);
-  double un[11];
-  double uon[3];
-  const double* ub = gen + gen_uplane(pos_pad(M));
+  typedef float v4f __attribute__((ext_vector_type(4)));
+  const double* mrow = gen_mean_row(p, b);
+  float en[12], eon[3];
+  double mn = mrow[j0];
+  auto stage_ld = [&](int jj) {
 #pragma unroll
-  for (int c = 0; c < 11; ++c) un[c] = ub[size_t(j0) * kGenRow + c];
+    for (int k = 0; k < 3; ++k) {
+      const v4f f = *reinterpret_cast<const v4f*>(st + jj * 12 + 4 * k);
 #pragma unroll
-  for (int i = 0; i < 3; ++i) uon[i] = ub[size_t(j0) * kGenRow + q + 4 * i];
+      for (int w = 0; w < 4; ++w) en[4 * k + w] = f[w];
+    }
+#pragma unroll
+    for (int i = 0; i < 3; ++i) eon[i] = st[jj * 12 + q + 4 * i];
+  };
+  stage_ld(0);
   for (int j = j0; j < j1; ++j) {
     double u[11], uo[3];
 #pragma unroll
-    for (int c = 0; c < 11; ++c) u[c] = un[c];
+    for (int c = 0; c < 11; ++c) u[c] = gen_u(en[c], mn);
 #pragma unroll
-    for (int i = 0; i < 3; ++i) uo[i] = uon[i];
+    for (int i = 0; i < 3; ++i) uo[i] = gen_u(eon[i], mn);
     const int jn = min(j + 1, j1 - 1);
-#pragma unroll
-    for (int c = 0; c < 11; ++c) un[c] = ub[size_t(jn) * kGenRow + c];
-#pragma unroll
-    for (int i = 0; i < 3; ++i) uon[i] = ub[size_t(jn) * kGenRow + q + 4 * i];
+    mn = mrow[jn];
+    stage_ld(jn - j0);
     double v[3], part = 0.0;
 #pragma unroll
     for (int i = 0; i < 3; ++i) {
@@ -88,21 +115,22 @@
   }
 }
 
-__global__ __launch_bounds__(256) __attribute__((amdgpu_waves_per_eu(2))) void k_bgen(Params p) {
+__global__ __launch_bounds__(256) __attribute__((amdgpu_waves_per_eu(2))) void k_bgen(Params p, int tb) {
   const int nblk = (p.M + 1 + 15) / 16;
   const int gq = (blockIdx.x * blockDim.x + tidx()) >> 2;
   const bool live = gq < p.nb * nblk;
   const int gqc = live ? gq : p.nb * nblk - 1;
-  bgen_quad(p, p.b0 + gqc / nblk, gqc % nblk, live);
+  __shared__ __attribute__((aligned(16))) float stage[64 * kGenStage];
+  bgen_quad(p, tb, p.b0 + gqc / nblk, gqc % nblk, live, stage + (tidx() >> 2) * kGenStage);
 }
 
 constexpr int kGenWaveWaves = 4;
-__global__ __launch_bounds__(64 * kGenWaveWaves) void k_bgen_wave(Params p) {
+__global__ __launch_bounds__(64 * kGenWaveWaves) void k_bgen_wave(Params p, int tb) {
   __shared__ double xl[kGenWaveWaves][32];
   const int nblk = (p.M + 1 + 15) / 16;
   const int w = tidx() >> 6, gw = blockIdx.x * kGenWaveWaves + w;
   if (gw >= p.nb * nblk) return;
-  bgen_wave(p, p.b0 + gw / nblk, gw % nblk, xl[w]);
+  bgen_wave(p, tb, p.b0 + gw / nblk, gw % nblk, xl[w]);
 }
 
 __global__ __launch_bounds__(kThreads) void k_bsigma(Params p, int tb) {
@@ -123,9 +151,9 @@
   const int nblk = (p.M + 1 + 15) / 16;
   if (p.gen_wave)
     hipLaunchKernelGGL(k_bgen_wave, dim3((p.nb * nblk + kGenWaveWaves - 1) / kGenWaveWaves), dim3(64 * kGenWaveWaves), 0,
-                       s, p);
+                       s, p, tb);
   else
-    hipLaunchKernelGGL(k_bgen, dim3((p.nb * nblk * 4 + 255) / 256), dim3(256), 0, s, p);
+    hipLaunchKernelGGL(k_bgen, dim3((p.nb * nblk * 4 + 255) / 256), dim3(256), 0, s, p, tb);
   if (tb == kBetaIters - 1) hipLaunchKernelGGL(k_bsigma, dim3(p.nb), dim3(kThreads), 0, s, p, tb);
 }
 
diff --git a/mpc-mmd_amd/csrc/k_bsample.hip b/mpc-mmd_amd/csrc/k_bsample.hip
--- a/mpc-mmd_amd/csrc/k_bsample.hip
+++ b/mpc-mmd_amd/csrc/k_bsample.hip
@@ -30,13 +30,14 @@
   const float* z = p.beta_z + size_t(tb - 1) * Pp * kBzCols;
   const int ys = ygen_stride(M);
   float* plane = p.ygen + size_t(b) * kBzCols * ys;
-  d4 S[TPW], Sp[TPW], Ya[TPW], Yb[TPW];
+  const float* E = gen_elites(p, tb, b);
+  d4 S[TPW], Sp[TPW];
 #pragma unroll
   for (int t = 0; t < TPW; ++t) {
     S[t] = Sp[t] = d4{0.0, 0.0, 0.0, 0.0};
     Sp[t][2] = h == 3 ? 1.0 : 0.0;
   }
-  const int nblk = Pp >> 4, cl = sample_chunk(nblk);
+  const int cl = sample_chunk(Pp >> 4);
   const __amdgpu_buffer_rsrc_t yr = ygen_rsrc(plane, ys);
   const int vl = (2 * h * ys + r) * 4, v43 = h == 0 ? vl : kDropOffset;
   auto store = [&](const d4* Yv, int q0) {
@@ -45,34 +46,18 @@
     else
       block_store<TPW>(Yv, plane, q0, M, ys, s0, r, h);
   };
-  SampleBlock<TPW> qa, qb;
-  const SampleRsrc srs = sample_rsrc(G, gm, z, Pp, r, h);
+  const SampleRsrc srs = sample_rsrc(G, E, gm, z, M, r, h);
   auto load = [&](SampleBlock<TPW>& q, int q0) {
     if constexpr (TPW == kSampleTiles)
       load_block_buf(q, srs, q0);
     else
-      load_block(q, G, G + gen_uplane(Pp), gm, z, q0, s0, r, h);
+      load_block(q, G, E, gen_mean_row(p, b), gm, z, M, q0, s0, r, h);
   };
-  load(qa, 0);
-  for (int c = 0; c < nblk; c += 2) {
-    const int p0 = c << 4;
-    load(qb, p0 + 16);
-    __builtin_amdgcn_sched_barrier(0);
-    block_mfma(qa, S, Sp, Ya, r, h);
-    __builtin_amdgcn_sched_barrier(0);
-    if (c > 0) store(Yb, p0 - 16);
-    __builtin_amdgcn_sched_barrier(0);
-    load(qa, min(p0 + 32, Pp - 16));
-    __builtin_amdgcn_sched_barrier(0);
-    block_mfma(qb, S, Sp, Yb, r, h);
+  walk_blocks<TPW>(0, sample_blocks(M), M, r, h, S, Sp, load, store, [&](int c) {
     if ((c + 2) % cl == 0)
 #pragma unroll
       for (int t = 0; t < TPW; ++t) fold_chunk(Sp[t], S[t]);
-    __builtin_amdgcn_sched_barrier(0);
-    store(Ya, p0);
-    __builtin_amdgcn_sched_barrier(0);
-  }
-  store(Yb, Pp - 16);
+  });
   MPCMMD_STAMP(p, 1);
 }
 
@@ -114,30 +99,17 @@
     for (int i = 0; i < 3; ++i) dS[k][i][lane] = Sl[i];
   }
   __syncthreads();
-  d4 S[1] = {d4{0.0, 0.0, 0.0, 0.0}}, Sp[1] = {d4{0.0, 0.0, 0.0, 0.0}}, Ya[1], Yb[1];
+  d4 S[1] = {d4{0.0, 0.0, 0.0, 0.0}}, Sp[1] = {d4{0.0, 0.0, 0.0, 0.0}};
   Sp[0][2] = h == 3 ? 1.0 : 0.0;
   for (int j = 0; j < k; ++j)
 #pragma unroll
     for (int i = 0; i < 3; ++i) Sp[0][i] = Sp[0][i] + dS[j][i][lane];
-  SampleBlock<1> qa, qb;
-  const int pend = c1 << 4;
-  load_block(qa, G, G + gen_uplane(Pp), gm, z, c0 << 4, s0, r, h);
-  for (int c = c0; c < c1; c += 2) {
-    const int p0 = c << 4;
-    load_block(qb, G, G + gen_uplane(Pp), gm, z, p0 + 16, s0, r, h);
-    __builtin_amdgcn_sched_barrier(0);
-    block_mfma(qa, S, Sp, Ya, r, h);
-    __builtin_amdgcn_sched_barrier(0);
-    if (c > c0) block_store<1>(Yb, plane, p0 - 16, M, ys, s0, r, h);
-    __builtin_amdgcn_sched_barrier(0);
-    load_block(qa, G, G + gen_uplane(Pp), gm, z, min(p0 + 32, pend - 16), s0, r, h);
-    __builtin_amdgcn_sched_barrier(0);
-    block_mfma(qb, S, Sp, Yb, r, h);
-    __builtin_amdgcn_sched_barrier(0);
-    block_store<1>(Ya, plane, p0, M, ys, s0, r, h);
-    __builtin_amdgcn_sched_barrier(0);
-  }
-  block_store<1>(Yb, plane, pend - 16, M, ys, s0, r, h);
+  const float* E = gen_elites(p, tb, b);
+  const double* mrow = gen_mean_row(p, b);
+  walk_blocks<1>(
+      c0, min(sample_blocks(M), c1), M, r, h, S, Sp,
+      [&](SampleBlock<1>& q, int q0) { load_block(q, G, E, mrow, gm, z, M, q0, s0, r, h); },
+      [&](const d4* Yv, int q0) { block_store<1>(Yv, plane, q0, M, ys, s0, r, h); }, [](int) {});
   MPCMMD_STAMP(p, 1);
 }
 
diff --git a/mpc-mmd_amd/csrc/layout.hpp b/mpc-mmd_amd/csrc/layout.hpp
--- a/mpc-mmd_amd/csrc/layout.hpp
+++ b/mpc-mmd_amd/csrc/layout.hpp
@@ -21,7 +21,10 @@
 constexpr int kGenRow = 12;
 constexpr int kGenStride = 2 * kGenRow;
 constexpr int kGenW = 0, kGenMean = 11;
-HDI_CONST size_t gen_uplane(int Pp) { return size_t(Pp) * kGenRow; }
+HDI_CONST size_t gen_means(int Pp) { return size_t(Pp) * kGenRow; }
+constexpr double kRsqrt10 = 0x1.43d136248490fp-2;
+HDI_CONST double gen_u(float e, double m) { return (double(e) - m) * kRsqrt10; }
+HDI_CONST double gen_mean_slot(double m) { return double(float(m)); }
 HDI_CONST int ygen_stride(int M) { return ((M + 1) + 31) & ~31; }
 constexpr int kBzCols = 96;
 HDI_CONST size_t bz_index(int j, int s) {
```

After: 145.8 steps/s, median of 6. 3.6% higher.
